# theislab/dca

Hardware: NVIDIA H100
Metric: cells/sec (ZINB AE epoch, device-timed) (higher is better)
Workload: dtype bf16-gemm/f32-acc/f32-loss

## Files before the change

dca_b200/_lib.py:

```python
from __future__ import annotations

import ctypes as C
import os

_HERE = os.path.dirname(os.path.abspath(__file__))
LIB_PATH = os.path.join(_HERE, "libdca_b200.so")

DCA_MAX_HIDDEN = 8
DCA_NAME_LEN = 48

ACTIVATION_IDS = {"relu": 0, "linear": 1, "elu": 2, "selu": 3, "tanh": 4, "sigmoid": 5, "hard_sigmoid": 6,
                  "softplus": 7, "softsign": 8, "exponential": 9, "LeakyReLU": 10, "PReLU": 11}
OPTIMIZERS = {"RMSprop": (0, 1e-3), "SGD": (1, 1e-2), "Adagrad": (2, 1e-2), "Adadelta": (3, 1.0), "Adam": (4, 1e-3),
              "Adamax": (5, 2e-3), "Nadam": (6, 2e-3)}
OPTIMIZERS.update({k.lower(): v for k, v in list(OPTIMIZERS.items())})
AE_TYPE_IDS = {"zinb-conddisp": 0, "zinb": 1, "nb-conddisp": 2, "nb": 3,
               "poisson": 4, "normal": 5, "nb-shared": 6, "zinb-shared": 7, "zinb-elempi": 8, "nb-fork": 9, "zinb-fork": 10}
F32, BF16 = 0, 1
GEMM_AUTO, GEMM_GENERIC, GEMM_TCGEN05 = 0, 1, 2
REGION_PARAMS, REGION_GRADS, REGION_RMS, REGION_BN_STATE, REGION_EPOCH_ACC = 0, 1, 2, 3, 4


class DcaError(RuntimeError):
    pass
# ... 59 lines not shown
    "dca_read_loss": (C.c_int, [_vp, C.POINTER(_f), C.POINTER(_i32), _vp]),
    "dca_read_epoch_acc": (C.c_int, [_vp, C.POINTER(C.c_double * 4), _i32, _vp]),
    "dca_train_step_host": (C.c_int, [_vp, _vp, _vp, _vp, _i32, _f, _f, C.POINTER(_f), _vp]),
    "dca_set_input_transform": (C.c_int, [_vp, _vp, _vp, _i32, _i32, _vp]),
    "dca_set_loss_ring": (C.c_int, [_vp, _vp, _i32]),
    "dca_stream_begin": (C.c_int, [_vp, _vp, _i64, _vp, _i64, _i32, _vp]),
    "dca_stream_begin_packed": (C.c_int, [_vp, _vp, _i32, _i64, _vp, _vp, _vp, _i64, _i32, _vp]),
    "dca_stream_begin_sparse": (C.c_int, [_vp, _vp, _vp, _vp, _vp, _vp, _vp, _i64, _i32, _vp]),
    "dca_stream_step": (C.c_int, [_vp, _i64, _i64, _vp]),
    "dca_stream_end": (C.c_int, [_vp, _vp]),
    "dca_expand_packed_counts": (C.c_int, [_vp, _i32, _vp, _vp, _vp, _i32, _i32, _vp, _vp, _i32, _i32, _vp, _vp, _i32, _vp,
                                           _vp]),
    "dca_expand_sparse_counts": (C.c_int, [_vp, _vp, _vp, _i32, _vp, _vp, _vp, _i32, _i32, _vp, _vp, _i32, _i32, _vp, _vp,
                                           _i32, _vp, _vp]),
    "dca_zinb_loss_fwd_bwd": (C.c_int, [_vp, _i64, _vp, _vp, _vp, _vp, _vp, _i64, _i32, _i32, _i32, _f, _f,
                                        _vp, _vp, _vp, _i32, _vp, _vp, _vp, _sz, _vp]),
    "dca_zinb_loss_workspace_bytes": (C.c_int, [_i32, _i32, C.POINTER(_sz)]),
    "dca_zinb_loss_fwd": (C.c_int, [_vp, _i64, _vp, _vp, _vp, _vp, _vp, _i64, _i32, _i32, _i32, _f,
                                    _vp, _vp, _sz, _vp]),
    "dca_zinb_elem_host": (C.c_int, [_i32, _f, _f, _f, _f, _f, _f, C.POINTER(_f * 4)]),
    "dca_dropout_mask_host": (C.c_int, [C.c_uint64, C.c_uint64, _i32, _i64, _f, _vp]),
    "dca_activation_host": (C.c_int, [_i32, _f, _f, C.POINTER(_f * 2)]),
    "dca_dense_heads_fwd": (C.c_int, [_vp, _i64, _i32, _i32, _i32, _vp, _vp, _vp, _vp, _vp, _vp, _vp,
                                      _vp, _vp, _vp, _i64, _vp]),
    "dca_tc_heads_fwd": (C.c_int, [_vp, _i32, _vp, _vp, _i32, _i32, C.POINTER(_i32 * 3), _vp, _vp, _vp, _vp, _i64, _vp]),
    "dca_tc_heads_loss": (C.c_int, [_vp, _i32, _vp, _vp, _i32, _vp, _i64, _vp, _vp, _f, _f, _vp, _vp, _vp, _i64, _vp,
                                    _vp, _sz, _vp]),
    "dca_tc_gene_gemm": (C.c_int, [_i32, _vp, _vp, _vp, _i64, _i32, _i32, _i32, _vp, _vp, _vp, _vp, _vp, _vp, _i64, _i32,
                                   _vp, _vp, _vp, _vp]),
    "dca_tc_gene_gemm_sms": (C.c_int, [_i32, _vp, _vp, _vp, _i64, _i32, _i32, _i32, _vp, _vp, _vp, _vp, _vp, _vp, _i64,
                                       _i32, _vp, _vp, _vp, _vp, _i32]),
    "dca_tc_gene_gemm_rows": (C.c_int, [_i32, _vp, _vp, _vp, _i64, _vp, _i32, _i32, _i32, _vp, _vp, _vp, _vp, _vp, _vp,
                                        _i64, _i32, _vp, _vp, _vp, _vp, _i32]),
    "dca_tc_probe": (C.c_int, [_vp, _i32, _i32, _vp, _i32, _i32, _i32, _i32, _i32, _i32, _i32, _i32, _i32, _i32, _i32,
                               _vp, _vp]),
    "dca_profile_enable": (C.c_int, [_vp, _i32]),
    "dca_profile_read": (C.c_int, [_vp, C.POINTER(C.c_double * 6), C.POINTER(C.c_int64 * 6), _i32]),
    "dca_engine_info": (C.c_int, [_vp, C.POINTER(_i32 * 8)]),
    "dca_write_text_matrix": (C.c_int, [C.c_char_p, _vp, _i32, _i64, _i64, _i64, _vp, _vp, _i32, _i32]),
    "dca_read_text_counts": (C.c_int, [C.c_char_p, _i32, _i32, _i64, _i32, _vp, _vp, _i64, _vp, _vp, _i64, _vp]),
    "dca_read_mtx_counts": (C.c_int, [C.c_char_p, _i32, _i64, _i32, _vp, _vp, _vp, _vp, _vp]),
    "dca_count_escapes": (C.c_int, [_vp, _i32, _i64, _i64, _i64, _vp, _i32]),
    "dca_pack_counts": (C.c_int, [_vp, _i32, _i64, _i64, _i64, _i32, _vp, _vp, _vp, _i32]),
    "dca_sparse_counts": (C.c_int, [_vp, _i32, _i64, _i64, _i64, _vp, _vp, _i32]),
    "dca_pack_sparse": (C.c_int, [_vp, _i32, _i64, _i64, _i64, _vp, _vp, _vp, _vp, _vp, _i32]),
    "dca_preprocess_workspace_bytes": (C.c_int, [_i64, _i32, C.POINTER(_sz)]),
    "dca_counts_csr_to_dense": (C.c_int, [_vp, _vp, _vp, _i64, _i32, _vp, _i64, _vp]),
    "dca_count_totals": (C.c_int, [_vp, _i64, _i64, _i32, _vp, _vp, _vp, _vp, _sz, _vp]),
    "dca_gather_counts": (C.c_int, [_vp, _i64, _vp, _i64, _vp, _i32, _vp, _i64, _vp]),
    "dca_log_moments": (C.c_int, [_vp, _i64, _i64, _i32, _vp, C.c_double, _i32, _vp, _vp, _vp, _sz, _vp]),
    "dca_normalize_write": (C.c_int, [_vp, _i64, _i64, _i32, _vp, C.c_double, _i32, _vp, _vp, _vp, _i32, _i64, _vp]),
    "dca_stats_workspace_bytes": (C.c_int, [_i64, _i32, _i64, C.POINTER(_sz)]),
    "dca_stats_begin": (C.c_int, [_i64, _i32, _vp, _sz, _vp]),
    "dca_count_totals_rows": (C.c_int, [_vp, _i64, _i64, _i64, _i64, _i32, _vp, _vp, _sz, _vp]),
    "dca_count_totals_finish": (C.c_int, [_i64, _i32, _vp, _vp, _vp, _sz, _vp]),
    "dca_log_moments_rows": (C.c_int, [_i32, _vp, _i64, _i64, _i64, _i64, _i32, _vp, C.c_double, _i32, _vp, _vp, _sz,
                                       _vp]),
    "dca_log_moments_finish": (C.c_int, [_i32, _i64, _i32, _i32, _vp, _vp, _sz, _vp]),
    "dca_set_input_transform_exact": (C.c_int, [_vp, _vp, _vp, C.c_double, _i32, _vp]),
    "dca_stream_row_totals": (C.c_int, [_vp, _vp]),
    "dca_stream_predict": (C.c_int, [_vp, _i64, _i64, _vp, _vp, _vp, _i64, _vp, _vp]),
    "dca_stream_eval": (C.c_int, [_vp, _i64, _i64, _vp]),
    "dca_stream_capacity": (C.c_int, [_vp, C.POINTER(_i64), C.POINTER(_i64)]),
    "dca_expand_packed_counts_exact": (C.c_int, [_vp, _i32, _vp, _vp, _vp, _i32, _i32, C.c_double, _i32, _vp, _vp, _vp,
                                                 _vp, _i32, _vp, _vp]),
    "dca_expand_sparse_counts_exact": (C.c_int, [_vp, _vp, _vp, _i32, _vp, _vp, _vp, _i32, _i32, C.c_double, _i32, _vp,
# ... 49 lines not shown
```

dca_b200/csrc/gene_gemm_tc.cu:

```cuda
#include "engine.h"
#include "tc_common.cuh"

namespace dca {
namespace tc {
int g_gg_profile = 0;
namespace gg {

constexpr int kThreads = 256;
constexpr uint32_t kZBytes = 128 * 128 * 2;
constexpr uint32_t kWBytes = 64 * 128 * 2;
constexpr uint32_t kHBytes = 128 * 64 * 2;
constexpr uint32_t kOutBytes = 128 * 64 * 4;
constexpr uint32_t kOnesBytes = 16 * 128;
constexpr int kMaxGb = 4;
constexpr int kMaxSlots = 16;

template <bool DO_A, bool DO_B>
constexpr int stages() { return DO_A && DO_B ? 2 : 3; }
template <bool DO_A, bool DO_B>
constexpr uint32_t stage_bytes() { return kZBytes + (DO_B ? kWBytes : 0) + (DO_A ? kHBytes : 0); }
template <bool DO_A, bool DO_B, bool COLSUM>
constexpr uint32_t smem_bytes() {
  return stages<DO_A, DO_B>() * stage_bytes<DO_A, DO_B>() + (DO_A ? kOutBytes : 0) + (COLSUM ? kOnesBytes : 0) + 1024;
}

struct Params {
  int B, G, n_heads;
  int n_cb, n_gb;
  int gb_per_item, cb_per_item;
  int gene_ranges, cell_splits;
  int total_items;
  float* db[3];
  float* part; int64_t part_stride;
  const int32_t* rows; const __nv_bfloat16* zsrc; int64_t ldz;
};

__device__ __forceinline__ void cp_async_16(uint32_t smem_dst, const void* src, uint32_t src_bytes) {
  asm volatile("cp.async.cg.shared.global [%0], [%1], 16, %2;" ::"r"(smem_dst), "l"(src), "r"(src_bytes) : "memory");
}
__device__ __forceinline__ void cp_async_commit() { asm volatile("cp.async.commit_group;" ::: "memory"); }
template <int N>
__device__ __forceinline__ void cp_async_wait() { asm volatile("cp.async.wait_group %0;" ::"n"(N) : "memory"); }

template <bool DO_A, bool DO_B, bool COLSUM, bool WK, int MAXG>
__global__ void __launch_bounds__(kThreads, 1)
gene_gemm_kernel(const __grid_constant__ CUtensorMap map_z0, const __grid_constant__ CUtensorMap map_z1,
                 const __grid_constant__ CUtensorMap map_z2, const __grid_constant__ CUtensorMap map_h,
                 const __grid_constant__ CUtensorMap map_w0, const __grid_constant__ CUtensorMap map_w1,
                 const __grid_constant__ CUtensorMap map_w2, const __grid_constant__ CUtensorMap map_dw0, const __grid_constant__ CUtensorMap map_dw1,
                 const __grid_constant__ CUtensorMap map_dw2, const int dw_transposed, const Params p) {
  constexpr int kStages = stages<DO_A, DO_B>();
  constexpr uint32_t kStage = stage_bytes<DO_A, DO_B>();
  extern __shared__ __align__(1024) uint8_t smem_raw[];
  uint8_t* smem = smem_raw + ((1024u - (smem_u32(smem_raw) & 1023u)) & 1023u);
  uint8_t* s_st = smem;
  float* s_o = reinterpret_cast<float*>(s_st + kStages * kStage);
  uint8_t* s_ones = reinterpret_cast<uint8_t*>(s_o) + (DO_A ? kOutBytes : 0);
  __shared__ uint64_t full[kStages];

  if (threadIdx.x == 0) {
    for (int i = 0; i < kStages; ++i) mbar_init(&full[i], 1);
    fence_barrier_init();
  }
  if (COLSUM) {
    for (int i = threadIdx.x; i < (int)kOnesBytes / 4; i += kThreads) reinterpret_cast<uint32_t*>(s_ones)[i] = 0x3F803F80u;
    fence_proxy_async_smem();
  }
  __syncthreads();

  const int wg = threadIdx.x >> 7, w = (threadIdx.x >> 5) & 3, l = threadIdx.x & 31;
  const int frow = 16 * w + (l >> 2), fcol = 2 * (l & 3);

  auto stage_begin = [&]() {
    if (threadIdx.x == 0) bulk_wait_read<0>();
    __syncthreads();
  };
  auto stage_end = [&](const CUtensorMap* m, int c0, int c1) {
    fence_proxy_async_smem();
    __syncthreads();
    if (threadIdx.x == 0) { tma_reduce_add_2d(m, c0, c1, s_o); bulk_commit(); }
  };

  uint32_t T0 = 0;
  const bool gather = p.rows != nullptr;
  const int g_rh = threadIdx.x >> 3, g_c = threadIdx.x & 7, g_h = g_rh & 1, g_r0 = g_rh >> 1;
  const uint32_t g_dst = g_h * (kZBytes / 2) + g_r0 * 128 + ((g_c ^ (g_r0 & 7)) << 4);
  int src_row[8];
  for (int item = blockIdx.x; item < p.total_items; item += gridDim.x) {
    const int cs = item % p.cell_splits, r = item / p.cell_splits;
    const int gr = r % p.gene_ranges, head = r / p.gene_ranges;
    const int gb0 = gr * p.gb_per_item, ng = min(p.n_gb, gb0 + p.gb_per_item) - gb0;
    const int cb0 = cs * p.cb_per_item, ncb = min(p.n_cb, cb0 + p.cb_per_item) - cb0;
    const int n_tiles = ng * ncb;
    const CUtensorMap* mz = head == 0 ? &map_z0 : (head == 1 ? &map_z1 : &map_z2);
    const CUtensorMap* mw = head == 0 ? &map_w0 : (head == 1 ? &map_w1 : &map_w2);
    const CUtensorMap* mdw = head == 0 ? &map_dw0 : (head == 1 ? &map_dw1 : &map_dw2);

    auto issue = [&](int t) {
      const int st = (T0 + t) % kStages;
      const int cb = cb0 + t / ng, gb = gb0 + t % ng;
      uint8_t* dst = s_st + st * kStage;
      mbar_expect_tx(&full[st], gather ? kStage - kZBytes : kStage);
      if (!gather) {
        tma_load_2d(dst, mz, gb * 128, cb * 128, &full[st]);
        tma_load_2d(dst + kZBytes / 2, mz, gb * 128 + 64, cb * 128, &full[st]);
      }
      if (DO_B) {
        if (WK) {
          tma_load_2d(dst + kZBytes, mw, gb * 128, 0, &full[st]);
          tma_load_2d(dst + kZBytes + kWBytes / 2, mw, gb * 128 + 64, 0, &full[st]);
        } else {
          tma_load_2d(dst + kZBytes, mw, 0, gb * 128, &full[st]);
        }
      }
      if (DO_A) tma_load_2d(dst + kZBytes + (DO_B ? kWBytes : 0), &map_h, 0, cb * 128, &full[st]);
    };
    auto load_rows = [&](int t) {
      const int cb = cb0 + t / ng;
#pragma unroll
      for (int i = 0; i < 8; ++i) {
        const int r = cb * 128 + g_r0 + 16 * i;
        src_row[i] = r < p.B ? __ldg(p.rows + r) : -1;
      }
    };
    auto copy_rows = [&](int t) {
      const int st = (T0 + t) % kStages, g0 = (gb0 + t % ng) * 128 + g_h * 64 + g_c * 8;
      const uint32_t gbytes = g0 < p.G ? (uint32_t)min(16, 2 * (p.G - g0)) : 0u;
      const uint32_t dst = smem_u32(s_st + st * kStage) + g_dst;
#pragma unroll
      for (int i = 0; i < 8; ++i) {
        const bool ok = src_row[i] >= 0 && gbytes != 0;
        cp_async_16(dst + i * 2048, ok ? p.zsrc + (int64_t)src_row[i] * p.ldz + g0 : p.zsrc, ok ? gbytes : 0u);
      }
      if (t + 1 < n_tiles) load_rows(t + 1);
    };
    if (gather) load_rows(0);
    for (int t = 0; t < kStages - 1; ++t) {
      if (t < n_tiles) {
        if (threadIdx.x == 0) issue(t);
        if (gather) copy_rows(t);
      }
      if (gather) cp_async_commit();
    }

    float acc_b[DO_B ? 32 : 1];
    float acc_a[DO_A ? MAXG : 1][32];
    float acc_c[COLSUM ? MAXG : 1][8];
#pragma unroll
    for (int j = 0; j < (DO_A ? MAXG : 1); ++j)
#pragma unroll
      for (int i = 0; i < 32; ++i) acc_a[j][i] = 0.f;
#pragma unroll
    for (int j = 0; j < (COLSUM ? MAXG : 1); ++j)
#pragma unroll
      for (int i = 0; i < 8; ++i) acc_c[j][i] = 0.f;

    int t = 0;
    for (int cbi = 0; cbi < ncb; ++cbi) {
      const int cb = cb0 + cbi;
#pragma unroll
      for (int i = 0; i < (DO_B ? 32 : 1); ++i) acc_b[i] = 0.f;
#pragma unroll
      for (int jj = 0; jj < (DO_A ? MAXG : 1); ++jj)
      for (int j = jj; j < (DO_A ? min(jj + 1, ng) : ng); ++j) {
        if (t + kStages - 1 < n_tiles) {
          if (threadIdx.x == 0) issue(t + kStages - 1);
          if (gather) copy_rows(t + kStages - 1);
        }
        if (gather) {
          cp_async_commit();
          cp_async_wait<kStages - 1>();
          fence_proxy_async_smem();
          __syncthreads();
        }
        const int st = (T0 + t) % kStages;
        mbar_wait(&full[st], ((T0 + t) / kStages) & 1);
        const uint32_t zb = smem_u32(s_st + st * kStage), wb = zb + kZBytes, hb = wb + (DO_B ? kWBytes : 0);
        wgmma_fence();
        if constexpr (DO_B) {
#pragma unroll
          for (int h = 0; h < 2; ++h)
#pragma unroll
            for (int k = 0; k < 4; ++k) {
              const uint64_t da = make_smem_desc(zb + h * (kZBytes / 2) + wg * 64 * 128 + k * 32, 0, 1024);
              if (WK) wgmma_m64n64k16<0, 0>(acc_b, da, make_smem_desc(wb + h * (kWBytes / 2) + k * 32, 0, 1024), 1u);
              else wgmma_m64n64k16<0, 1>(acc_b, da, make_smem_desc(wb + (h * 4 + k) * 2048, 0, 1024), 1u);
            }
        }
        if constexpr (DO_A) {
#pragma unroll
          for (int k = 0; k < 8; ++k) {
            const uint64_t da = make_smem_desc(zb + wg * (kZBytes / 2) + k * 2048, 0, 1024);
            wgmma_m64n64k16<1, 1>(acc_a[jj], da, make_smem_desc(hb + k * 2048, 0, 1024), 1u);
            if constexpr (COLSUM) wgmma_m64n16k16<1, 0>(acc_c[jj], da, make_smem_desc(smem_u32(s_ones) + (k & 3) * 32, 0, 1024), 1u);
          }
        }
        wgmma_commit();
        wgmma_wait<0>();
        if constexpr (DO_B) acc_fence(acc_b);
        if constexpr (DO_A) {
#pragma unroll
          for (int jj2 = 0; jj2 < MAXG; ++jj2) acc_fence(acc_a[jj2]);
        }
        if constexpr (COLSUM) {
#pragma unroll
          for (int jj2 = 0; jj2 < MAXG; ++jj2) acc_fence(acc_c[jj2]);
        }
        __syncthreads();
        ++t;
      }
      if constexpr (DO_B) {
        float* dst = p.part + (int64_t)(head * p.gene_ranges + gr) * p.part_stride + (int64_t)cb * 128 * 64;
#pragma unroll
        for (int i = 0; i < 32; i += 2) {
          const int row = wg * 64 + frow + 8 * ((i >> 1) & 1), col = 8 * (i >> 2) + fcol;
          *reinterpret_cast<float2*>(dst + row * 64 + col) = make_float2(acc_b[i], acc_b[i + 1]);
        }
      }
    }
    T0 += n_tiles;
    if constexpr (DO_A) {
#pragma unroll
      for (int j = 0; j < MAXG; ++j) {
        if (j >= ng) break;
        const int gb = gb0 + j;
        stage_begin();
        if (dw_transposed) {
#pragma unroll
          for (int i = 0; i < 32; ++i) {
            const int g = wg * 64 + frow + 8 * ((i >> 1) & 1), f = 8 * (i >> 2) + fcol + (i & 1);
            s_o[f * 128 + g] = acc_a[j][i];
          }
          stage_end(mdw, gb * 128, 0);
        } else {
#pragma unroll
          for (int i = 0; i < 32; i += 2) {
            const int g = wg * 64 + frow + 8 * ((i >> 1) & 1), f = 8 * (i >> 2) + fcol;
            *reinterpret_cast<float2*>(s_o + g * 64 + f) = make_float2(acc_a[j][i], acc_a[j][i + 1]);
          }
          stage_end(mdw, 0, gb * 128);
        }
        if constexpr (COLSUM) {
          float* dbh = head == 0 ? p.db[0] : (head == 1 ? p.db[1] : p.db[2]);
          if ((l & 3) == 0 && dbh) {
            const int g = gb * 128 + wg * 64 + frow;
            if (g < p.G) atomicAdd(dbh + g, acc_c[j][0]);
            if (g + 8 < p.G) atomicAdd(dbh + g + 8, acc_c[j][2]);
          }
        }
      }
    }
  }
  if (threadIdx.x == 0) bulk_wait<0>();
}

__global__ void gene_gemm_reduce_kernel(const float* __restrict__ part, int slots, int64_t stride, float* __restrict__ out,
                                        int64_t n) {
  const int64_t i = ((int64_t)blockIdx.x * blockDim.x + threadIdx.x) * 4;
  if (i >= n) return;
  float4 acc = *reinterpret_cast<const float4*>(out + i);
  for (int sl = 0; sl < slots; ++sl) {
    const float4 v = __ldcs(reinterpret_cast<const float4*>(part + sl * stride + i));
    acc.x += v.x; acc.y += v.y; acc.z += v.z; acc.w += v.w;
  }
  *reinterpret_cast<float4*>(out + i) = acc;
}

}

size_t gene_gemm_workspace_bytes(int B) { return sizeof(float) * (size_t)gg::kMaxSlots * cdiv(B, 128) * 128 * 64; }

int gene_gemm_tc(int mode, const __nv_bfloat16* const Z[3], int64_t ldz, const int32_t* rows, int B, int G, int n_heads,
                 const __nv_bfloat16* H, const __nv_bfloat16* const W[3], float* out_b, float* const dW[3], int64_t dW_ld,
                 int dW_transposed, float* const db[3], void* ws, size_t ws_bytes, int sm_count, cudaStream_t s) {
  using namespace gg;
  if (ldz % 8 != 0) { set_error("gene_gemm_tc: ldz must be a multiple of 8 (16-byte TMA stride)"); return DCA_ERR_BAD_ARG; }
  if (mode < 1 || mode > 3) { set_error("gene_gemm_tc: bad mode %d", mode); return DCA_ERR_BAD_ARG; }
  if (rows && (mode == 3 || n_heads != 1)) { set_error("gene_gemm_tc: row indices are for modes 1 and 2 (one Z)"); return DCA_ERR_BAD_ARG; }
  const bool do_a = mode & 2, do_b = mode & 1;
  if (do_b && (!ws || ws_bytes < gene_gemm_workspace_bytes(B))) { set_error("gene_gemm_tc: workspace too small"); return DCA_ERR_BAD_ARG; }
  CUtensorMap mz[3], mh, mw[3], mdw[3];
  for (int i = 0; i < 3; ++i) DCA_TRY(make_tensor_map_2d(&mz[i], Z[i < n_heads ? i : 0], 2, 1, (uint64_t)B, (uint64_t)G, (uint64_t)ldz, 128, 64, 1));
  mh = mz[0];
  for (int i = 0; i < 3; ++i) mw[i] = mdw[i] = mz[0];
  if (do_a) {
    DCA_TRY(make_tensor_map_2d(&mh, H, 2, 1, (uint64_t)B, 64, 64, 128, 64, 1));
    for (int i = 0; i < 3; ++i) {
      float* d = dW[i < n_heads ? i : 0];
      if (dW_transposed) DCA_TRY(make_tensor_map_2d(&mdw[i], d, 4, 0, 64, (uint64_t)G, (uint64_t)dW_ld, 64, 128, 0));
      else {
        if (dW_ld != 64) { set_error("gene_gemm_tc: non-transposed dW needs ld == 64"); return DCA_ERR_BAD_ARG; }
        DCA_TRY(make_tensor_map_2d(&mdw[i], d, 4, 0, (uint64_t)G, 64, 64, 128, 64, 0));
      }
    }
  }
  if (do_b) {
    for (int i = 0; i < 3; ++i) {
      const __nv_bfloat16* w = W[i < n_heads ? i : 0];
      if (mode == 3) DCA_TRY(make_tensor_map_2d(&mw[i], w, 2, 1, 64, (uint64_t)G, (uint64_t)G, 64, 64, 1));
      else DCA_TRY(make_tensor_map_2d(&mw[i], w, 2, 1, (uint64_t)G, 64, 64, 128, 64, 1));
    }
  }
  Params base{};
  base.B = B; base.G = G; base.n_heads = n_heads;
  base.n_cb = cdiv(B, 128); base.n_gb = cdiv(G, 128);
  for (int i = 0; i < 3; ++i) base.db[i] = db ? db[i] : nullptr;
  base.part = reinterpret_cast<float*>(ws); base.part_stride = (int64_t)base.n_cb * 128 * 64;
  base.rows = rows; base.zsrc = Z[0]; base.ldz = ldz;

#define DCA_GG_LAUNCH(P, A, Bb, Cc, WKk, MG)                                                                           \
  do {                                                                                                                 \
    static bool attr = false;                                                                                          \
    constexpr uint32_t sm = smem_bytes<A, Bb, Cc>();                                                                       \
    if (!attr) { DCA_CUDA_OK(cudaFuncSetAttribute(gene_gemm_kernel<A, Bb, Cc, WKk, MG>, cudaFuncAttributeMaxDynamicSharedMemorySize, (int)sm)); attr = true; } \
    gene_gemm_kernel<A, Bb, Cc, WKk, MG><<<min(P.total_items, sm_count), kThreads, sm, s>>>(mz[0], mz[1], mz[2], mh, mw[0], mw[1], mw[2],      \
                                                                          mdw[0], mdw[1], mdw[2], dW_transposed, P);  \
    DCA_LAUNCH_CHECK();                                                                                                \
  } while (0)

  if (do_a) {
    Params p = base;
    int best_gpi = 1; long long best_cost = -1;
    for (int gpi = 1; gpi <= kMaxGb; ++gpi) {
      const long long items = (long long)cdiv(p.n_gb, gpi) * n_heads, rounds = (items + sm_count - 1) / sm_count;
      const long long cost = rounds * ((long long)gpi * p.n_cb + 2ll * gpi);
      if (best_cost < 0 || cost < best_cost) { best_cost = cost; best_gpi = gpi; }
    }
    p.gb_per_item = best_gpi; p.gene_ranges = cdiv(p.n_gb, best_gpi);
    p.cb_per_item = p.n_cb; p.cell_splits = 1;
    p.total_items = p.gene_ranges * n_heads;
    if (mode == 3) DCA_GG_LAUNCH(p, true, false, true, false, kMaxGb);
    else DCA_GG_LAUNCH(p, true, false, false, false, kMaxGb);
  }
  if (do_b) {
    Params p = base;
    p.cb_per_item = 1; p.cell_splits = p.n_cb;
    int gsplits = cdiv(4 * sm_count, p.n_cb * n_heads); if (gsplits < 1) gsplits = 1;
    if (gsplits > kMaxSlots / n_heads) gsplits = kMaxSlots / n_heads;
    if (gsplits > p.n_gb) gsplits = p.n_gb;
    while (gsplits > 1 && cdiv(p.n_gb, gsplits) < 4) --gsplits;
    p.gb_per_item = cdiv(p.n_gb, gsplits); p.gene_ranges = cdiv(p.n_gb, p.gb_per_item);
    p.total_items = p.gene_ranges * p.cell_splits * n_heads;
    if (mode == 3) DCA_GG_LAUNCH(p, false, true, false, true, 1);
    else DCA_GG_LAUNCH(p, false, true, false, false, 1);
    const int64_t n = (int64_t)B * 64;
    gene_gemm_reduce_kernel<<<(unsigned)cdiv(n / 4, 256), 256, 0, s>>>(p.part, p.gene_ranges * n_heads, p.part_stride, out_b, n);
    DCA_LAUNCH_CHECK();
  }
#undef DCA_GG_LAUNCH
  return DCA_OK;
}

}
}

using namespace dca;
extern "C" int dca_tc_gene_gemm_rows(int32_t mode, const void* Z0, const void* Z1, const void* Z2, int64_t ldz,
                                     const int32_t* rows, int32_t batch, int32_t genes, int32_t n_heads, const void* H,
                                     const void* W, float* out_b, float* dW0, float* dW1, float* dW2, int64_t dW_ld,
                                     int32_t dW_transposed, float* db0, float* db1, float* db2, void* stream, int32_t sm_count) {
  if (!Z0 || batch <= 0 || genes <= 0 || n_heads < 1 || n_heads > 3) { set_error("dca_tc_gene_gemm: bad argument"); return DCA_ERR_BAD_ARG; }
  int dev = 0, sms = 132;
  cudaGetDevice(&dev);
  cudaDeviceGetAttribute(&sms, cudaDevAttrMultiProcessorCount, dev);
  if (sm_count > 0 && sm_count < sms) sms = sm_count;
  const __nv_bfloat16* Z[3] = {(const __nv_bfloat16*)Z0, (const __nv_bfloat16*)Z1, (const __nv_bfloat16*)Z2};
  float* dW[3] = {dW0, dW1, dW2};
  float* db[3] = {db0, db1, db2};
  const __nv_bfloat16* Wp[3];
  for (int i = 0; i < 3; ++i) Wp[i] = (const __nv_bfloat16*)W + (mode == 3 ? (size_t)(i < n_heads ? i : 0) * 64 * genes : 0);
  cudaStream_t st = (cudaStream_t)stream;
  const size_t ws_bytes = tc::gene_gemm_workspace_bytes(batch);
  void* ws = nullptr;
  DCA_CUDA_OK(cudaMallocAsync(&ws, ws_bytes, st));
  const int rc = tc::gene_gemm_tc(mode, Z, ldz, rows, batch, genes, n_heads, (const __nv_bfloat16*)H, Wp, out_b, dW,
                                  dW_ld, dW_transposed, db, ws, ws_bytes, sms, st);
  DCA_CUDA_OK(cudaFreeAsync(ws, st));
  return rc;
}
extern "C" int dca_tc_gene_gemm_sms(int32_t mode, const void* Z0, const void* Z1, const void* Z2, int64_t ldz,
                                    int32_t batch, int32_t genes, int32_t n_heads, const void* H, const void* W, float* out_b,
                                    float* dW0, float* dW1, float* dW2, int64_t dW_ld, int32_t dW_transposed, float* db0,
                                    float* db1, float* db2, void* stream, int32_t sm_count) {
  return dca_tc_gene_gemm_rows(mode, Z0, Z1, Z2, ldz, nullptr, batch, genes, n_heads, H, W, out_b, dW0, dW1, dW2, dW_ld,
                               dW_transposed, db0, db1, db2, stream, sm_count);
}
extern "C" int dca_tc_gene_gemm(int32_t mode, const void* Z0, const void* Z1, const void* Z2, int64_t ldz, int32_t batch,
                                int32_t genes, int32_t n_heads, const void* H, const void* W, float* out_b, float* dW0,
                                float* dW1, float* dW2, int64_t dW_ld, int32_t dW_transposed, float* db0, float* db1,
                                float* db2, void* stream) {
  return dca_tc_gene_gemm_sms(mode, Z0, Z1, Z2, ldz, batch, genes, n_heads, H, W, out_b, dW0, dW1, dW2, dW_ld,
                              dW_transposed, db0, db1, db2, stream, 0);
}
```

dca_b200/csrc/zinb_loss.cu:

```cuda
#include "dca_internal.cuh"
#include <string>
#include "zinb_math.cuh"
#include "tc_common.cuh"
#include "head_act.cuh"
#include <cstdlib>

namespace dca {
namespace tc { extern int g_gg_profile; }

namespace {

constexpr int kThreads = 256;
constexpr int kVec = 4;
constexpr int kColsPerBlock = kThreads * kVec;
constexpr int kMaxBlocks = 65536;

struct LossTune { int target_blocks; unsigned producer_sleep_ns, consumer_sleep_ns; int branch_free; int ring; };
LossTune g_tune = {0 , 0u, 0u, 1 ,
                   1 };

int sm_count_cached() {
  static int n = 0;
  if (!n) { int dev = 0; if (cudaGetDevice(&dev) != cudaSuccess || cudaDeviceGetAttribute(&n, cudaDevAttrMultiProcessorCount, dev) != cudaSuccess || n <= 0) n = 132; }
  return n;
}

struct Plan { int col_blocks, rows_per_block, row_chunks; };

inline Plan make_plan(int B, int G, int cols_per_block, int max_rpb = 1 << 30) {
  Plan p;
  p.col_blocks = cdiv(G, cols_per_block);
  const int target = g_tune.target_blocks > 0 ? g_tune.target_blocks
                     : ((long long)B * G <= (32ll << 20) ? 3 * sm_count_cached() : 16 * sm_count_cached());
  int chunks = target / p.col_blocks;
  if (chunks < 1) chunks = 1;
  if (chunks > B) chunks = B;
  int rpb = cdiv(B, chunks);
  if (rpb < 2 && B >= 2) rpb = 2;
  if (rpb > max_rpb) rpb = max_rpb;
  while ((long long)cdiv(B, rpb) * p.col_blocks > kMaxBlocks && rpb < max_rpb) ++rpb;
  p.rows_per_block = rpb;
// ... 1080 lines not shown
  for (int i = 0; i < 3; ++i) { p.bias[i] = a.bias[i]; p.dz[i] = a.dz[i]; }
  p.Y = a.Y; p.ldy = a.ldy; p.rows = a.rows; p.sf = a.sf; p.B = B; p.G = G; p.ldz = a.ldz;
  p.nblk = cdiv(B, 64);
  const long long units = (long long)cdiv(G, 128) * p.nblk;
  if (units > INT_MAX) { set_error("heads_loss_tc: %lld (gene tile, cell block) units, over 2^31 - 1", units); return DCA_ERR_BAD_ARG; }
  p.units = (int)units;
  p.ridge = a.ridge; p.inv_n = a.inv_n;
  p.loss_partial = reinterpret_cast<double*>(a.ws); p.lf = lf_dev;
  FoldArgs fa{reinterpret_cast<unsigned*>(reinterpret_cast<char*>(a.ws) + sizeof(double) * (size_t)kMaxBlocks), a.loss_sum,
              a.fin_penalty, a.fin_loss_slot, a.fin_epoch_acc, a.fin_batch};
  if (!a.counter_ready) DCA_CUDA_OK(cudaMemsetAsync(fa.counter, 0, sizeof(unsigned), s));
  static bool attr = false;
  if (!attr) { DCA_CUDA_OK(cudaFuncSetAttribute(heads_loss_kernel, cudaFuncAttributeMaxDynamicSharedMemorySize, (int)kSmemBytes)); attr = true; }
  const int grid = (int)std::min<long long>(p.units, sm_count_cached());
  heads_loss_kernel<<<grid, kCtaThreads, kSmemBytes, s>>>(mh, mw[0], mw[1], mw[2], p, fa);
  DCA_LAUNCH_CHECK();
  return DCA_OK;
}

}

using namespace dca;

extern "C" int dca_set_tunable(const char* name, int64_t value) {
  if (!name) { set_error("dca_set_tunable: null name"); return DCA_ERR_BAD_ARG; }
  const std::string n(name);
  if (n == "loss_target_blocks" && value >= 0 && value <= kMaxBlocks) g_tune.target_blocks = (int)value;
  else if (n == "loss_producer_sleep_ns" && value >= 0 && value <= 100000) g_tune.producer_sleep_ns = (unsigned)value;
  else if (n == "loss_consumer_sleep_ns" && value >= 0 && value <= 100000) g_tune.consumer_sleep_ns = (unsigned)value;
  else if (n == "fused_heads" && (value == 0 || value == 1)) g_fused_heads_default = (int)value;
  else if (n == "loss_branch_free" && (value == 0 || value == 1)) g_tune.branch_free = (int)value;
  else if (n == "loss_ring" && value >= 0 && value <= 2) g_tune.ring = (int)value;
  else if (n == "gg_profile" && (value == 0 || value == 1)) tc::g_gg_profile = (int)value;
  else { set_error("dca_set_tunable: unknown name or value out of range (%s = %lld)", name, (long long)value); return DCA_ERR_BAD_ARG; }
  return DCA_OK;
}

extern "C" int dca_zinb_loss_workspace_bytes(int32_t batch, int32_t genes, size_t* bytes) {
  if (!bytes || batch <= 0 || genes <= 0) { set_error("dca_zinb_loss_workspace_bytes: bad argument"); return DCA_ERR_BAD_ARG; }
  *bytes = loss_workspace_bytes(batch, genes);
  return DCA_OK;
}

extern "C" int dca_zinb_loss_fwd_bwd(const float* Y, int64_t ldy, const int32_t* rows, const float* sf,
                                     const float* m, const float* d, const float* pi, int64_t ld,
                                     int32_t batch, int32_t genes, int32_t ae_type, float ridge, float inv_n,
                                     void* dzm, void* dzd, void* dzp, int32_t grad_dtype, float* dtheta,
                                     double* loss_sum, void* workspace, size_t workspace_bytes, void* stream) {
  if (ae_type < 0 || ae_type > 3) { set_error("dca_zinb_loss_fwd_bwd: unknown ae_type %d", ae_type); return DCA_ERR_BAD_ARG; }
  LossArgs a{Y, ldy, rows, sf, m, d, pi, ld, batch, genes, ae_type, ridge, inv_n, dzm, dzd, dzp,
             grad_dtype == DCA_BF16 ? 1 : 0, dtheta, loss_sum, workspace, workspace_bytes};
  return zinb_loss_fwd_bwd(a, (cudaStream_t)stream);
}

extern "C" int dca_tc_heads_loss(const void* Hb, int32_t batch, const void* Wk, const float* bias, int32_t genes,
                                 const float* Y, int64_t ldy, const int32_t* rows, const float* sf, float ridge, float inv_n,
                                 void* dzm, void* dzd, void* dzp, int64_t ldz, double* loss_sum, void* workspace,
                                 size_t workspace_bytes, void* stream) {
  if (!Hb || !Wk || !bias || !Y || !dzm || !dzd || !dzp || !loss_sum || batch <= 0 || genes <= 0) {
    set_error("dca_tc_heads_loss: bad argument"); return DCA_ERR_BAD_ARG;
  }
  HeadsLossArgs a{};
  a.H3 = (const __nv_bfloat16*)Hb; a.B = batch; a.G = genes;
  for (int i = 0; i < 3; ++i) { a.W[i] = (const __nv_bfloat16*)Wk + (size_t)i * 64 * genes; a.bias[i] = bias + (size_t)i * genes; }
  a.Y = Y; a.ldy = ldy; a.rows = rows; a.sf = sf; a.ridge = ridge; a.inv_n = inv_n;
  a.dz[0] = (__nv_bfloat16*)dzm; a.dz[1] = (__nv_bfloat16*)dzd; a.dz[2] = (__nv_bfloat16*)dzp; a.ldz = ldz;
// ... 65 lines not shown
```

include/dca_b200.h:

```cpp
#ifndef DCA_B200_H
#define DCA_B200_H

#include <stddef.h>
#include <stdint.h>

#ifdef __cplusplus
extern "C" {
#endif

#define DCA_B200_VERSION 100
#define DCA_MAX_HIDDEN 8
#define DCA_NAME_LEN 48

typedef enum dca_status {
  DCA_OK = 0,
  DCA_ERR_BAD_ARG = -1,
  DCA_ERR_CUDA = -2,
  DCA_ERR_UNSUPPORTED = -3,
  DCA_ERR_NONFINITE = -4,
  DCA_ERR_NO_DEVICE = -5
} dca_status;

typedef enum dca_ae_type {
  DCA_AE_ZINB_CONDDISP = 0,
// ... 207 lines not shown
                       float out[4]);

int dca_dropout_mask_host(uint64_t seed, uint64_t step, int32_t layer, int64_t n, float rate, uint8_t* keep);
int dca_activation_host(int32_t act, float x, float alpha, float out[2]);

int dca_dense_heads_fwd(const float* H, int64_t ldh, int32_t batch, int32_t K, int32_t genes,
                        const float* w_mean, const float* b_mean,
                        const float* w_disp, const float* b_disp,
                        const float* w_pi, const float* b_pi,
                        const float* row_scale,
                        float* m_out, float* d_out, float* pi_out, int64_t ld_out, void* stream);

int dca_tc_heads_fwd(const void* Hb, int32_t batch, const void* Wk, const float* bias, int32_t genes,
                     int32_t n_heads, const int32_t kind[3], const float* row_scale,
                     float* out0, float* out1, float* out2, int64_t ld_out, void* stream);

int dca_tc_heads_loss(const void* Hb, int32_t batch, const void* Wk, const float* bias, int32_t genes,
                      const float* Y, int64_t ldy, const int32_t* rows, const float* sf, float ridge, float inv_n,
                      void* dzm, void* dzd, void* dzp, int64_t ldz, double* loss_sum, void* workspace,
                      size_t workspace_bytes, void* stream);

int dca_tc_gene_gemm(int32_t mode, const void* Z0, const void* Z1, const void* Z2, int64_t ldz, int32_t batch,
                     int32_t genes, int32_t n_heads, const void* H, const void* W, float* out_b,
                     float* dW0, float* dW1, float* dW2, int64_t dW_ld, int32_t dW_transposed,
                     float* db0, float* db1, float* db2, void* stream);
int dca_tc_gene_gemm_sms(int32_t mode, const void* Z0, const void* Z1, const void* Z2, int64_t ldz, int32_t batch,
                         int32_t genes, int32_t n_heads, const void* H, const void* W, float* out_b,
                         float* dW0, float* dW1, float* dW2, int64_t dW_ld, int32_t dW_transposed,
                         float* db0, float* db1, float* db2, void* stream, int32_t sm_count);
int dca_tc_gene_gemm_rows(int32_t mode, const void* Z0, const void* Z1, const void* Z2, int64_t ldz, const int32_t* rows,
                          int32_t batch, int32_t genes, int32_t n_heads, const void* H, const void* W, float* out_b,
                          float* dW0, float* dW1, float* dW2, int64_t dW_ld, int32_t dW_transposed,
                          float* db0, float* db1, float* db2, void* stream, int32_t sm_count);

#define DCA_PRE_SIZE_FACTORS 1
#define DCA_PRE_LOG1P 2
#define DCA_PRE_SCALE 4
int dca_preprocess_workspace_bytes(int64_t n_cells, int32_t genes, size_t* bytes);
int dca_counts_csr_to_dense(const int64_t* indptr, const int32_t* indices, const float* data, int64_t n_cells,
                            int32_t genes, float* Y, int64_t ldy, void* stream);
int dca_count_totals(const float* Y, int64_t ldy, int64_t n_cells, int32_t genes, double* cell_totals,
                     double* gene_totals, int64_t* n_bad, void* workspace, size_t workspace_bytes, void* stream);
int dca_gather_counts(const float* Y, int64_t ldy, const int32_t* rows, int64_t n_rows, const int32_t* cols,
                      int32_t n_cols, float* out, int64_t ldo, void* stream);
int dca_log_moments(const float* Y, int64_t ldy, int64_t n_cells, int32_t genes, const double* n_counts, double median,
                    int32_t flags, double* mean, double* std, void* workspace, size_t workspace_bytes, void* stream);
int dca_normalize_write(const float* Y, int64_t ldy, int64_t n_cells, int32_t genes, const double* n_counts,
                        double median, int32_t flags, const double* mean, const double* std, void* X, int32_t x_dtype,
                        int64_t ldx, void* stream);
int dca_stats_workspace_bytes(int64_t n_cells, int32_t genes, int64_t max_chunk_rows, size_t* bytes);
int dca_stats_begin(int64_t n_cells, int32_t genes, void* workspace, size_t workspace_bytes, void* stream);
int dca_count_totals_rows(const float* Y, int64_t ldy, int64_t row0, int64_t n_rows, int64_t n_cells, int32_t genes,
                          double* cell_totals, void* workspace, size_t workspace_bytes, void* stream);
int dca_count_totals_finish(int64_t n_cells, int32_t genes, double* gene_totals, int64_t* n_bad, void* workspace,
                            size_t workspace_bytes, void* stream);
int dca_log_moments_rows(int32_t pass, const float* Y, int64_t ldy, int64_t row0, int64_t n_rows, int64_t n_cells,
                         int32_t genes, const double* n_counts, double median, int32_t flags, const double* mean,
                         void* workspace, size_t workspace_bytes, void* stream);
int dca_log_moments_finish(int32_t pass, int64_t n_cells, int32_t genes, int32_t flags, double* out, void* workspace,
                           size_t workspace_bytes, void* stream);

int dca_tc_probe(const void* A, int32_t a_rows, int32_t a_cols, const void* B, int32_t b_rows, int32_t b_cols,
                 int32_t a_mn_major, int32_t b_mn_major, int32_t M, int32_t N, int32_t K,
                 int32_t a_lbo, int32_t a_sbo, int32_t b_lbo, int32_t b_sbo, float* D, void* stream);

#define DCA_N_PHASES 6
// ... 34 lines not shown
```

Baseline: 2.846 million.

## Fuse head-backward dW and dH passes into one banded launch with staggered starts

In mode 3 the separate (a) weight-gradient launch and (b) input-gradient launch are replaced by a single persistent launch. Its item list interleaves per-gene-block (a) items and per-cell-block (b) items in bands, so both kinds of work share Z tiles while they are still in L2. Blocks start after a clock-based stagger proportional to their position in the band, which is meant to space out TMA traffic to the same tiles. This removes one kernel launch and the tail between the two passes. In exchange, the banded path uses 3 stages of Z+W shape for both kinds, adds spin-wait delays at startup, and adds a schedule-inspection API.

```diff
diff --git a/dca_b200/_lib.py b/dca_b200/_lib.py
--- a/dca_b200/_lib.py
+++ b/dca_b200/_lib.py
@@ -115,6 +115,7 @@
                                        _i32, _vp, _vp, _vp, _vp, _i32]),
     "dca_tc_gene_gemm_rows": (C.c_int, [_i32, _vp, _vp, _vp, _i64, _vp, _i32, _i32, _i32, _vp, _vp, _vp, _vp, _vp, _vp,
                                         _i64, _i32, _vp, _vp, _vp, _vp, _i32]),
+    "dca_head_bwd_schedule": (C.c_int, [_i32, _i32, _i32, _i32, _i32, _vp, _i64, C.POINTER(_i64), _vp]),
     "dca_tc_probe": (C.c_int, [_vp, _i32, _i32, _vp, _i32, _i32, _i32, _i32, _i32, _i32, _i32, _i32, _i32, _i32, _i32,
                                _vp, _vp]),
     "dca_profile_enable": (C.c_int, [_vp, _i32]),
diff --git a/dca_b200/csrc/gene_gemm_tc.cu b/dca_b200/csrc/gene_gemm_tc.cu
--- a/dca_b200/csrc/gene_gemm_tc.cu
+++ b/dca_b200/csrc/gene_gemm_tc.cu
@@ -4,6 +4,8 @@
 namespace dca {
 namespace tc {
 int g_gg_profile = 0;
+int g_head_bwd_banded = 1;
+int g_head_bwd_stagger = 1300;
 namespace gg {
 
 constexpr int kThreads = 256;
@@ -15,13 +17,30 @@
 constexpr int kMaxGb = 4;
 constexpr int kMaxSlots = 16;
 
-template <bool DO_A, bool DO_B>
-constexpr int stages() { return DO_A && DO_B ? 2 : 3; }
-template <bool DO_A, bool DO_B>
-constexpr uint32_t stage_bytes() { return kZBytes + (DO_B ? kWBytes : 0) + (DO_A ? kHBytes : 0); }
-template <bool DO_A, bool DO_B, bool COLSUM>
+static_assert(kWBytes == kHBytes, "the two item kinds of the banded launch share one stage shape");
+template <bool DO_A, bool DO_B, bool BANDED>
+constexpr int stages() { return DO_A && DO_B && !BANDED ? 2 : 3; }
+template <bool DO_A, bool DO_B, bool BANDED>
+constexpr uint32_t stage_bytes() { return BANDED ? kZBytes + kWBytes : kZBytes + (DO_B ? kWBytes : 0) + (DO_A ? kHBytes : 0); }
+template <bool DO_A, bool DO_B, bool COLSUM, bool BANDED>
 constexpr uint32_t smem_bytes() {
-  return stages<DO_A, DO_B>() * stage_bytes<DO_A, DO_B>() + (DO_A ? kOutBytes : 0) + (COLSUM ? kOnesBytes : 0) + 1024;
+  return stages<DO_A, DO_B, BANDED>() * stage_bytes<DO_A, DO_B, BANDED>() + (DO_A ? kOutBytes : 0) + (COLSUM ? kOnesBytes : 0) + 1024;
+}
+
+struct BandItem { int kind, head, gr, gb0, ng, cb0, ncb; };
+
+__host__ __device__ inline BandItem band_item(int k, int n_gb, int n_cb, int gpr, int ranges) {
+  const int per_head = n_gb + ranges * n_cb, full_band = gpr + n_cb;
+  BandItem it;
+  it.head = k / per_head; k -= it.head * per_head;
+  it.gr = min(k / full_band, ranges - 1); k -= it.gr * full_band;
+  const int gb0 = it.gr * gpr, ng = min(n_gb, gb0 + gpr) - gb0, m = min(ng, n_cb);
+  int idx;
+  if (k < 2 * m) { it.kind = k & 1; idx = k >> 1; }
+  else { it.kind = ng > n_cb ? 0 : 1; idx = k - m; }
+  if (it.kind == 0) { it.gb0 = gb0 + idx; it.ng = 1; it.cb0 = 0; it.ncb = n_cb; }
+  else { it.gb0 = gb0; it.ng = ng; it.cb0 = idx; it.ncb = 1; }
+  return it;
 }
 
 struct Params {
@@ -30,6 +49,7 @@
   int gb_per_item, cb_per_item;
   int gene_ranges, cell_splits;
   int total_items;
+  int stagger;
   float* db[3];
   float* part; int64_t part_stride;
   const int32_t* rows; const __nv_bfloat16* zsrc; int64_t ldz;
@@ -42,15 +62,17 @@
 template <int N>
 __device__ __forceinline__ void cp_async_wait() { asm volatile("cp.async.wait_group %0;" ::"n"(N) : "memory"); }
 
-template <bool DO_A, bool DO_B, bool COLSUM, bool WK, int MAXG>
+template <bool DO_A, bool DO_B, bool COLSUM, bool WK, int MAXG, bool BANDED>
 __global__ void __launch_bounds__(kThreads, 1)
 gene_gemm_kernel(const __grid_constant__ CUtensorMap map_z0, const __grid_constant__ CUtensorMap map_z1,
                  const __grid_constant__ CUtensorMap map_z2, const __grid_constant__ CUtensorMap map_h,
                  const __grid_constant__ CUtensorMap map_w0, const __grid_constant__ CUtensorMap map_w1,
                  const __grid_constant__ CUtensorMap map_w2, const __grid_constant__ CUtensorMap map_dw0, const __grid_constant__ CUtensorMap map_dw1,
                  const __grid_constant__ CUtensorMap map_dw2, const int dw_transposed, const Params p) {
-  constexpr int kStages = stages<DO_A, DO_B>();
-  constexpr uint32_t kStage = stage_bytes<DO_A, DO_B>();
+  static_assert(!BANDED || (DO_A && DO_B && MAXG == 1), "banded items hold one gene block of (a) accumulators");
+  constexpr int kStages = stages<DO_A, DO_B, BANDED>();
+  constexpr uint32_t kStage = stage_bytes<DO_A, DO_B, BANDED>();
+  constexpr uint32_t kHOff = kZBytes + (DO_B && !BANDED ? kWBytes : 0);
   extern __shared__ __align__(1024) uint8_t smem_raw[];
   uint8_t* smem = smem_raw + ((1024u - (smem_u32(smem_raw) & 1023u)) & 1023u);
   uint8_t* s_st = smem;
@@ -86,11 +108,30 @@
   const int g_rh = threadIdx.x >> 3, g_c = threadIdx.x & 7, g_h = g_rh & 1, g_r0 = g_rh >> 1;
   const uint32_t g_dst = g_h * (kZBytes / 2) + g_r0 * 128 + ((g_c ^ (g_r0 & 7)) << 4);
   int src_row[8];
+  if constexpr (BANDED) {
+    if (p.stagger > 0 && blockIdx.x < p.total_items) {
+      const BandItem it = band_item(blockIdx.x, p.n_gb, p.n_cb, p.gb_per_item, p.gene_ranges);
+      const long long wait = (long long)(it.kind ? it.cb0 : it.gb0 - it.gr * p.gb_per_item) * p.stagger;
+      if (threadIdx.x == 0) {
+        const long long c0 = clock64();
+        while (clock64() - c0 < wait) __nanosleep(100);
+      }
+      __syncthreads();
+    }
+  }
   for (int item = blockIdx.x; item < p.total_items; item += gridDim.x) {
-    const int cs = item % p.cell_splits, r = item / p.cell_splits;
-    const int gr = r % p.gene_ranges, head = r / p.gene_ranges;
-    const int gb0 = gr * p.gb_per_item, ng = min(p.n_gb, gb0 + p.gb_per_item) - gb0;
-    const int cb0 = cs * p.cb_per_item, ncb = min(p.n_cb, cb0 + p.cb_per_item) - cb0;
+    int head, gr, gb0, ng, cb0, ncb;
+    bool ia = DO_A, ib = DO_B;
+    if constexpr (BANDED) {
+      const BandItem it = band_item(item, p.n_gb, p.n_cb, p.gb_per_item, p.gene_ranges);
+      head = it.head; gr = it.gr; gb0 = it.gb0; ng = it.ng; cb0 = it.cb0; ncb = it.ncb;
+      ia = it.kind == 0; ib = !ia;
+    } else {
+      const int cs = item % p.cell_splits, r = item / p.cell_splits;
+      gr = r % p.gene_ranges; head = r / p.gene_ranges;
+      gb0 = gr * p.gb_per_item; ng = min(p.n_gb, gb0 + p.gb_per_item) - gb0;
+      cb0 = cs * p.cb_per_item; ncb = min(p.n_cb, cb0 + p.cb_per_item) - cb0;
+    }
     const int n_tiles = ng * ncb;
     const CUtensorMap* mz = head == 0 ? &map_z0 : (head == 1 ? &map_z1 : &map_z2);
     const CUtensorMap* mw = head == 0 ? &map_w0 : (head == 1 ? &map_w1 : &map_w2);
@@ -105,7 +146,7 @@
         tma_load_2d(dst, mz, gb * 128, cb * 128, &full[st]);
         tma_load_2d(dst + kZBytes / 2, mz, gb * 128 + 64, cb * 128, &full[st]);
       }
-      if (DO_B) {
+      if (DO_B && ib) {
         if (WK) {
           tma_load_2d(dst + kZBytes, mw, gb * 128, 0, &full[st]);
           tma_load_2d(dst + kZBytes + kWBytes / 2, mw, gb * 128 + 64, 0, &full[st]);
@@ -113,7 +154,7 @@
           tma_load_2d(dst + kZBytes, mw, 0, gb * 128, &full[st]);
         }
       }
-      if (DO_A) tma_load_2d(dst + kZBytes + (DO_B ? kWBytes : 0), &map_h, 0, cb * 128, &full[st]);
+      if (DO_A && ia) tma_load_2d(dst + kHOff, &map_h, 0, cb * 128, &full[st]);
     };
     auto load_rows = [&](int t) {
       const int cb = cb0 + t / ng;
@@ -162,7 +203,7 @@
       for (int i = 0; i < (DO_B ? 32 : 1); ++i) acc_b[i] = 0.f;
 #pragma unroll
       for (int jj = 0; jj < (DO_A ? MAXG : 1); ++jj)
-      for (int j = jj; j < (DO_A ? min(jj + 1, ng) : ng); ++j) {
+      for (int j = jj; j < (DO_A && ia ? min(jj + 1, ng) : ng); ++j) {
         if (t + kStages - 1 < n_tiles) {
           if (threadIdx.x == 0) issue(t + kStages - 1);
           if (gather) copy_rows(t + kStages - 1);
@@ -175,9 +216,10 @@
         }
         const int st = (T0 + t) % kStages;
         mbar_wait(&full[st], ((T0 + t) / kStages) & 1);
-        const uint32_t zb = smem_u32(s_st + st * kStage), wb = zb + kZBytes, hb = wb + (DO_B ? kWBytes : 0);
+        const uint32_t zb = smem_u32(s_st + st * kStage), wb = zb + kZBytes, hb = zb + kHOff;
         wgmma_fence();
         if constexpr (DO_B) {
+          if (ib)
 #pragma unroll
           for (int h = 0; h < 2; ++h)
 #pragma unroll
@@ -188,6 +230,7 @@
             }
         }
         if constexpr (DO_A) {
+          if (ia)
 #pragma unroll
           for (int k = 0; k < 8; ++k) {
             const uint64_t da = make_smem_desc(zb + wg * (kZBytes / 2) + k * 2048, 0, 1024);
@@ -209,7 +252,7 @@
         __syncthreads();
         ++t;
       }
-      if constexpr (DO_B) {
+      if constexpr (DO_B) if (ib) {
         float* dst = p.part + (int64_t)(head * p.gene_ranges + gr) * p.part_stride + (int64_t)cb * 128 * 64;
 #pragma unroll
         for (int i = 0; i < 32; i += 2) {
@@ -219,7 +262,7 @@
       }
     }
     T0 += n_tiles;
-    if constexpr (DO_A) {
+    if (DO_A && ia) {
 #pragma unroll
       for (int j = 0; j < MAXG; ++j) {
         if (j >= ng) break;
@@ -264,6 +307,33 @@
     acc.x += v.x; acc.y += v.y; acc.z += v.z; acc.w += v.w;
   }
   *reinterpret_cast<float4*>(out + i) = acc;
+}
+
+void plan_a(Params& p, int n_heads, int sm_count) {
+  int best_gpi = 1; long long best_cost = -1;
+  for (int gpi = 1; gpi <= kMaxGb; ++gpi) {
+    const long long items = (long long)cdiv(p.n_gb, gpi) * n_heads, rounds = (items + sm_count - 1) / sm_count;
+    const long long cost = rounds * ((long long)gpi * p.n_cb + 2ll * gpi);
+    if (best_cost < 0 || cost < best_cost) { best_cost = cost; best_gpi = gpi; }
+  }
+  p.gb_per_item = best_gpi; p.gene_ranges = cdiv(p.n_gb, best_gpi);
+  p.cb_per_item = p.n_cb; p.cell_splits = 1;
+  p.total_items = p.gene_ranges * n_heads;
+}
+void plan_b(Params& p, int n_heads, int sm_count) {
+  p.cb_per_item = 1; p.cell_splits = p.n_cb;
+  int gsplits = cdiv(4 * sm_count, p.n_cb * n_heads); if (gsplits < 1) gsplits = 1;
+  if (gsplits > kMaxSlots / n_heads) gsplits = kMaxSlots / n_heads;
+  if (gsplits > p.n_gb) gsplits = p.n_gb;
+  while (gsplits > 1 && cdiv(p.n_gb, gsplits) < 4) --gsplits;
+  p.gb_per_item = cdiv(p.n_gb, gsplits); p.gene_ranges = cdiv(p.n_gb, p.gb_per_item);
+  p.total_items = p.gene_ranges * p.cell_splits * n_heads;
+}
+void plan_banded(Params& p, int n_heads, int sm_count, int* grid) {
+  plan_b(p, n_heads, sm_count);
+  p.total_items = n_heads * (p.n_gb + p.gene_ranges * p.n_cb);
+  const int band = p.gb_per_item + p.n_cb;
+  *grid = min(p.total_items, sm_count >= band ? sm_count / band * band : sm_count);
 }
 
 }
@@ -308,41 +378,40 @@
   base.part = reinterpret_cast<float*>(ws); base.part_stride = (int64_t)base.n_cb * 128 * 64;
   base.rows = rows; base.zsrc = Z[0]; base.ldz = ldz;
 
-#define DCA_GG_LAUNCH(P, A, Bb, Cc, WKk, MG)                                                                           \
+#define DCA_GG_LAUNCH(P, GRID, A, Bb, Cc, WKk, MG, BND)                                                                \
   do {                                                                                                                 \
     static bool attr = false;                                                                                          \
-    constexpr uint32_t sm = smem_bytes<A, Bb, Cc>();                                                                       \
-    if (!attr) { DCA_CUDA_OK(cudaFuncSetAttribute(gene_gemm_kernel<A, Bb, Cc, WKk, MG>, cudaFuncAttributeMaxDynamicSharedMemorySize, (int)sm)); attr = true; } \
-    gene_gemm_kernel<A, Bb, Cc, WKk, MG><<<min(P.total_items, sm_count), kThreads, sm, s>>>(mz[0], mz[1], mz[2], mh, mw[0], mw[1], mw[2],      \
+    constexpr uint32_t sm = smem_bytes<A, Bb, Cc, BND>();                                                              \
+    if (!attr) { DCA_CUDA_OK(cudaFuncSetAttribute(gene_gemm_kernel<A, Bb, Cc, WKk, MG, BND>, cudaFuncAttributeMaxDynamicSharedMemorySize, (int)sm)); attr = true; } \
+    gene_gemm_kernel<A, Bb, Cc, WKk, MG, BND><<<GRID, kThreads, sm, s>>>(mz[0], mz[1], mz[2], mh, mw[0], mw[1], mw[2],  \
                                                                           mdw[0], mdw[1], mdw[2], dW_transposed, P);  \
     DCA_LAUNCH_CHECK();                                                                                                \
   } while (0)
 
+  if (mode == 3 && g_head_bwd_banded) {
+    Params p = base;
+    int grid = 0;
+    plan_banded(p, n_heads, sm_count, &grid);
+    p.stagger = g_head_bwd_stagger;
+    DCA_GG_LAUNCH(p, grid, true, true, true, true, 1, true);
+    const int64_t n = (int64_t)B * 64;
+    gene_gemm_reduce_kernel<<<(unsigned)cdiv(n / 4, 256), 256, 0, s>>>(p.part, p.gene_ranges * n_heads, p.part_stride, out_b, n);
+    DCA_LAUNCH_CHECK();
+    return DCA_OK;
+  }
   if (do_a) {
     Params p = base;
-    int best_gpi = 1; long long best_cost = -1;
-    for (int gpi = 1; gpi <= kMaxGb; ++gpi) {
-      const long long items = (long long)cdiv(p.n_gb, gpi) * n_heads, rounds = (items + sm_count - 1) / sm_count;
-      const long long cost = rounds * ((long long)gpi * p.n_cb + 2ll * gpi);
-      if (best_cost < 0 || cost < best_cost) { best_cost = cost; best_gpi = gpi; }
-    }
-    p.gb_per_item = best_gpi; p.gene_ranges = cdiv(p.n_gb, best_gpi);
-    p.cb_per_item = p.n_cb; p.cell_splits = 1;
-    p.total_items = p.gene_ranges * n_heads;
-    if (mode == 3) DCA_GG_LAUNCH(p, true, false, true, false, kMaxGb);
-    else DCA_GG_LAUNCH(p, true, false, false, false, kMaxGb);
+    plan_a(p, n_heads, sm_count);
+    const int grid = min(p.total_items, sm_count);
+    if (mode == 3) DCA_GG_LAUNCH(p, grid, true, false, true, false, kMaxGb, false);
+    else DCA_GG_LAUNCH(p, grid, true, false, false, false, kMaxGb, false);
   }
   if (do_b) {
     Params p = base;
-    p.cb_per_item = 1; p.cell_splits = p.n_cb;
-    int gsplits = cdiv(4 * sm_count, p.n_cb * n_heads); if (gsplits < 1) gsplits = 1;
-    if (gsplits > kMaxSlots / n_heads) gsplits = kMaxSlots / n_heads;
-    if (gsplits > p.n_gb) gsplits = p.n_gb;
-    while (gsplits > 1 && cdiv(p.n_gb, gsplits) < 4) --gsplits;
-    p.gb_per_item = cdiv(p.n_gb, gsplits); p.gene_ranges = cdiv(p.n_gb, p.gb_per_item);
-    p.total_items = p.gene_ranges * p.cell_splits * n_heads;
-    if (mode == 3) DCA_GG_LAUNCH(p, false, true, false, true, 1);
-    else DCA_GG_LAUNCH(p, false, true, false, false, 1);
+    plan_b(p, n_heads, sm_count);
+    const int grid = min(p.total_items, sm_count);
+    if (mode == 3) DCA_GG_LAUNCH(p, grid, false, true, false, true, 1, false);
+    else DCA_GG_LAUNCH(p, grid, false, true, false, false, 1, false);
     const int64_t n = (int64_t)B * 64;
     gene_gemm_reduce_kernel<<<(unsigned)cdiv(n / 4, 256), 256, 0, s>>>(p.part, p.gene_ranges * n_heads, p.part_stride, out_b, n);
     DCA_LAUNCH_CHECK();
@@ -392,3 +461,44 @@
   return dca_tc_gene_gemm_sms(mode, Z0, Z1, Z2, ldz, batch, genes, n_heads, H, W, out_b, dW0, dW1, dW2, dW_ld,
                               dW_transposed, db0, db1, db2, stream, 0);
 }
+extern "C" int dca_head_bwd_schedule(int32_t batch, int32_t genes, int32_t n_heads, int32_t sm_count, int32_t banded,
+                                     int32_t* items, int64_t cap, int64_t* n_items, int32_t* grid) {
+  if (batch <= 0 || genes <= 0 || n_heads < 1 || n_heads > 3 || sm_count < 1 || !n_items || !grid) {
+    set_error("dca_head_bwd_schedule: bad argument"); return DCA_ERR_BAD_ARG;
+  }
+  tc::gg::Params base{};
+  base.n_cb = cdiv(batch, 128); base.n_gb = cdiv(genes, 128);
+  int64_t k = 0;
+  auto put = [&](int launch, int kind, int head, int gb0, int ng, int cb0, int ncb, int slot) {
+    if (items && k < cap) {
+      int32_t* r = items + 8 * k;
+      r[0] = launch; r[1] = kind; r[2] = head; r[3] = gb0; r[4] = ng; r[5] = cb0; r[6] = ncb; r[7] = slot;
+    }
+    ++k;
+  };
+  if (banded) {
+    tc::gg::Params p = base;
+    plan_banded(p, n_heads, sm_count, &grid[0]);
+    grid[1] = 0;
+    for (int i = 0; i < p.total_items; ++i) {
+      const tc::gg::BandItem it = tc::gg::band_item(i, p.n_gb, p.n_cb, p.gb_per_item, p.gene_ranges);
+      put(0, it.kind, it.head, it.gb0, it.ng, it.cb0, it.ncb, it.kind ? it.head * p.gene_ranges + it.gr : -1);
+    }
+  } else {
+    tc::gg::Params pa = base, pb = base;
+    plan_a(pa, n_heads, sm_count);
+    plan_b(pb, n_heads, sm_count);
+    grid[0] = std::min(pa.total_items, (int)sm_count); grid[1] = std::min(pb.total_items, (int)sm_count);
+    for (int pass = 0; pass < 2; ++pass) {
+      const tc::gg::Params& p = pass ? pb : pa;
+      for (int i = 0; i < p.total_items; ++i) {
+        const int cs = i % p.cell_splits, r = i / p.cell_splits, gr = r % p.gene_ranges, head = r / p.gene_ranges;
+        const int gb0 = gr * p.gb_per_item, cb0 = cs * p.cb_per_item;
+        put(pass, pass, head, gb0, std::min(p.n_gb, gb0 + p.gb_per_item) - gb0, cb0, std::min(p.n_cb, cb0 + p.cb_per_item) - cb0,
+            pass ? head * p.gene_ranges + gr : -1);
+      }
+    }
+  }
+  *n_items = k;
+  return DCA_OK;
+}
diff --git a/dca_b200/csrc/zinb_loss.cu b/dca_b200/csrc/zinb_loss.cu
--- a/dca_b200/csrc/zinb_loss.cu
+++ b/dca_b200/csrc/zinb_loss.cu
@@ -6,7 +6,7 @@
 #include <cstdlib>
 
 namespace dca {
-namespace tc { extern int g_gg_profile; }
+namespace tc { extern int g_gg_profile; extern int g_head_bwd_banded; extern int g_head_bwd_stagger; }
 
 namespace {
 
@@ -1153,6 +1153,8 @@
   else if (n == "loss_branch_free" && (value == 0 || value == 1)) g_tune.branch_free = (int)value;
   else if (n == "loss_ring" && value >= 0 && value <= 2) g_tune.ring = (int)value;
   else if (n == "gg_profile" && (value == 0 || value == 1)) tc::g_gg_profile = (int)value;
+  else if (n == "head_bwd_banded" && (value == 0 || value == 1)) tc::g_head_bwd_banded = (int)value;
+  else if (n == "head_bwd_stagger" && value >= 0 && value <= 100000) tc::g_head_bwd_stagger = (int)value;
   else { set_error("dca_set_tunable: unknown name or value out of range (%s = %lld)", name, (long long)value); return DCA_ERR_BAD_ARG; }
   return DCA_OK;
 }
diff --git a/include/dca_b200.h b/include/dca_b200.h
--- a/include/dca_b200.h
+++ b/include/dca_b200.h
@@ -263,6 +263,8 @@
                           int32_t batch, int32_t genes, int32_t n_heads, const void* H, const void* W, float* out_b,
                           float* dW0, float* dW1, float* dW2, int64_t dW_ld, int32_t dW_transposed,
                           float* db0, float* db1, float* db2, void* stream, int32_t sm_count);
+int dca_head_bwd_schedule(int32_t batch, int32_t genes, int32_t n_heads, int32_t sm_count, int32_t banded,
+                          int32_t* items, int64_t cap, int64_t* n_items, int32_t* grid);
 
 #define DCA_PRE_SIZE_FACTORS 1
 #define DCA_PRE_LOG1P 2
```

After: 3.117 million, median of 6. +9.5%, better.
